# qiyunzhu/woltka

Measured on AMD Instinct MI355X. Metric: alignment records/sec classified, higher is better.
Workload: dtype u8; 1 GPU; synthetic SAM text of 50M reads x <=16 hits (10.50 GB) resident in HBM, 2M-node taxonomy, ranks phylum,genus,species: device tokenizer per 64 MB block + one weighted histogram per sample (the kernels of `woltka classify`, host link left out); records_per_gpu=250034804, reads_per_gpu=50000000

## Files before the change

### include/woltka_hip_measure.h

```cpp
#ifndef WOLTKA_HIP_MEASURE_H
#define WOLTKA_HIP_MEASURE_H
#include "woltka_hip.h"
#ifdef __cplusplus
extern "C" {
#endif

int wk_tune(wk_ctx* ctx, const char* name, int64_t value);

int wk_timer_begin(wk_ctx* ctx);
int wk_timer_end(wk_ctx* ctx);
int wk_timer_ms(wk_ctx* ctx, double* ms);
int wk_profile_kernels(wk_ctx* ctx, int enable);
int wk_last_kernel_ms(wk_ctx* ctx, const char* family, double* ms);

int wk_text_upload(wk_ctx* ctx, const char* text, int64_t begin, int64_t stop);
int wk_text_clear(wk_ctx* ctx);
int wk_dtok_fused_counts(wk_ctx* ctx, int64_t* done, int64_t* handed_back);
int wk_ordinal_chunk_counts(wk_ctx* ctx, int64_t* sorted, int64_t* gathered);
int wk_h2d_rate(wk_ctx* ctx, int64_t bytes, int reps, double* bytes_per_s);

#ifdef __cplusplus
}
#endif
#endif
```

### woltka_amd/_native.py

```python
import ctypes as C
import os
from fractions import Fraction

import numpy as np

_HERE = os.path.dirname(os.path.abspath(__file__))
LIB_PATH = os.environ.get('WOLTKA_HIP_LIB') or os.path.join(
    _HERE, 'libwoltka_hip.so')

ABI_VERSION = 5
OK, E_HIP, E_ARG, E_STATE, E_CAPACITY, E_RANGE, E_TABLE_FULL = (
    0, -1, -2, -3, -4, -5, -6)
KEY_FEATURE_BITS, KEY_GROUP_BITS, KEY_K_BITS, KEY_JOB_BITS = 28, 21, 12, 3
MAX_JOBS, MAX_K = 8, 4095
FEATURE_UNASSIGNED, MAX_FEATURE = 0x0FFFFFFF, 0x0FFFFFFE
MODE_NONE, MODE_FREE, MODE_RANK = 0, 1, 2
F_UNIQ, F_ABOVE, F_SUBOK, F_UNASSIGNED, F_SIZED = 1, 2, 4, 8, 16
ASSIGN_NONE, ASSIGN_MULTI, ASSIGN_EMPTY = -1, -2, -3
SUBJ_IS_SET, SUBJ_INDEXED, GROUP_UNIFORM = 1, 2, 4
MAX_RANK_SLOTS = MAX_JOBS * 4

SYMBOLS = (
    'wk_abi_version', 'wk_build_id', 'wk_device_count', 'wk_device_pci_bus_id',
    'wk_create', 'wk_destroy',
# ... 19 lines not shown
    'wk_tok_fetch', 'wk_tok_fetch_packed', 'wk_tok_set_subject_map',
    'wk_tok_read', 'wk_tok_trim', 'wk_tok_sam_span', 'wk_tok_span', 'wk_tok_set_header_state',
    'wk_dtok_format',
    'wk_dtok_copy', 'wk_dtok_copy_ahead', 'wk_dtok_copy_wait',
    'wk_dtok_copy_drop', 'wk_dtok_subject_map', 'wk_dtok_ahead_room', 'wk_dtok_text_back', 'wk_dtok_expect', 'wk_dtok_scan', 'wk_dtok_emit', 'wk_dtok_stage_hits', 'wk_dtok_stage_hits_append',
    'wk_dtok_scan_emit', 'wk_dtok_scan_emit_begin', 'wk_dtok_scan_emit_end',
    'wk_dtok_keep_reads', 'wk_readmap_tables',
    'wk_cover_begin', 'wk_dtok_cover_append', 'wk_cover_add',
    'wk_cover_finish', 'wk_cover_fetch', 'wk_cover_reset',
    'wk_dtok_readmap',
    'wk_dtok_readmap_fetch', 'wk_strata_load', 'wk_strata_labels',
    'wk_strata_groups', 'wk_strata_clear',
    'wk_demux_begin', 'wk_demux_pending', 'wk_demux_register',
    'wk_dtok_stage_reads', 'wk_demux_fetch', 'wk_dtok_stage_hits_demux',
    'wk_dtok_stage_reads_strata', 'wk_chunk_groups',
    'wk_dtok_stage_reads_plain', 'wk_classify_staged_keep',
    'wk_readmap_reads_tables', 'wk_dtok_readmap_reads',
    'wk_tok_subjects',
    'wk_tok_new_subjects', 'wk_tok_fetch_groups', 'wk_tok_strata_clear',
    'wk_tok_strata_load', 'wk_tok_strata_labels', 'wk_tok_strata_select',
    'wk_tok_strata_swap', 'wk_format_readmap',
    'wk_tok_fetch_samples', 'wk_tok_new_samples', 'wk_preorder',
    'wk_hier_create', 'wk_hier_destroy', 'wk_hier_last_error',
    'wk_hier_add_text', 'wk_hier_update', 'wk_hier_finish', 'wk_hier_arrays',
    'wk_hier_root', 'wk_hier_lookup', 'wk_hier_node_names', 'wk_hier_get',
    'wk_hier_size', 'wk_hier_keys', 'wk_hier_ranks',
    'wk_coords_parse', 'wk_coords_error', 'wk_coords_sizes',
    'wk_coords_fetch', 'wk_coords_free',
    'wk_gz_bound', 'wk_gz_member', 'wk_crc32', 'wk_gz_inflate_members',
    'wk_inflate_members_device', 'wk_dtok_inflate_ahead',
    'wk_gz_walk_members',
    'wk_gunzip_open', 'wk_gunzip_read', 'wk_gunzip_error', 'wk_gunzip_close',
    'wk_text_upload', 'wk_text_clear', 'wk_h2d_rate',
    'wk_dtok_fused_counts', 'wk_ordinal_chunk_counts')


class Job(C.Structure):
    _fields_ = [('mode', C.c_int32), ('rank_slot', C.c_int32),
                ('flags', C.c_uint32), ('_pad', C.c_uint32),
                ('major', C.c_double)]


class Stats(C.Structure):
    _fields_ = [('n_reads', C.c_int64), ('n_records', C.c_int64),
                ('n_pairs', C.c_int64), ('table_used', C.c_int64)]


_lib = None


def load_library():
    global _lib
    if _lib is not None:
        return _lib
    if not os.path.isfile(LIB_PATH):
        raise RuntimeError(
            f'{LIB_PATH} is missing: build it with `python -c "import '
            '__graft_entry__ as g; g.build()"` (hipcc --offload-arch=gfx950). '
            'There is no CPU fallback.')
    lib = C.CDLL(LIB_PATH)
    p = C.c_void_p
    i32p, i64p, u32p, u64p = (C.POINTER(C.c_int32), C.POINTER(C.c_int64),
                              C.POINTER(C.c_uint32), C.POINTER(C.c_uint64))
    proto = {
        'wk_abi_version': (C.c_int, []),
        'wk_build_id': (C.c_char_p, []),
        'wk_device_count': (C.c_int, []),
# ... 188 lines not shown
                                     i64p, C.POINTER(C.c_uint8), C.c_int64]),
        'wk_hier_finish': (C.c_int, [p, i64p, i32p]),
        'wk_hier_arrays': (C.c_int, [p, i32p, i32p, i32p, i32p]),
        'wk_hier_root': (C.c_int, [p, i32p]),
        'wk_hier_lookup': (C.c_int, [p, C.c_char_p, i64p, C.c_int64, i32p]),
        'wk_hier_node_names': (C.c_int, [p, i32p, C.c_int64, C.c_void_p,
                                         C.c_int64, i64p]),
        'wk_hier_get': (C.c_int, [p, C.c_int, C.c_char_p, C.c_int64,
                                  C.c_void_p, C.c_int64, i64p]),
        'wk_hier_size': (C.c_int64, [p, C.c_int]),
        'wk_hier_keys': (C.c_int, [p, C.c_int, C.c_void_p, C.c_int64, i64p]),
        'wk_hier_ranks': (C.c_int, [p, C.c_void_p, C.c_int64, i64p, i64p]),
        'wk_coords_parse': (C.c_int, [C.c_void_p, C.c_int64, C.POINTER(p)]),
        'wk_coords_error': (C.c_char_p, [p]),
        'wk_coords_sizes': (C.c_int, [p, i32p, i32p, i64p, i64p,
                                      C.POINTER(C.c_int)]),
        'wk_coords_fetch': (C.c_int, [p, i32p, i32p, i32p, i32p, C.c_void_p,
                                      i64p, C.c_void_p, i64p]),
        'wk_coords_free': (None, [p]),
        'wk_gz_bound': (C.c_int64, [C.c_int64]),
        'wk_gz_member': (C.c_int64, [C.c_void_p, C.c_int64, C.c_void_p,
                                     C.c_int64]),
        'wk_crc32': (C.c_uint32, [C.c_uint32, C.c_void_p, C.c_int64]),
        'wk_gz_inflate_members': (C.c_int64, [C.c_void_p, i64p, i64p, C.c_int64,
                                              C.c_void_p, i64p, C.c_int]),
        'wk_gunzip_open': (p, [C.c_char_p, C.c_int, C.c_char_p, C.c_size_t]),
        'wk_gunzip_read': (C.c_int64, [p, C.c_void_p, C.c_int64]),
        'wk_gunzip_error': (C.c_char_p, [p]),
        'wk_gunzip_close': (None, [p]),
        'wk_text_upload': (C.c_int, [p, C.c_void_p, C.c_int64, C.c_int64]),
        'wk_text_clear': (C.c_int, [p]),
        'wk_dtok_fused_counts': (C.c_int, [p, i64p, i64p]),
        'wk_ordinal_chunk_counts': (C.c_int, [p, i64p, i64p]),
        'wk_h2d_rate': (C.c_int, [p, C.c_int64, C.c_int,
                                  C.POINTER(C.c_double)]),
    }
    for name, (res, args) in proto.items():
        fn = getattr(lib, name)
        fn.restype = res
        fn.argtypes = args
    if lib.wk_abi_version() != ABI_VERSION:
        raise RuntimeError('libwoltka_hip.so ABI version mismatch')
    _lib = lib
    return lib


def _arr(a, dtype):
    return np.ascontiguousarray(a, dtype=dtype)


def _ptr(a, ctype):
    return None if a is None else a.ctypes.data_as(C.POINTER(ctype))


def device_pci_bus_id(device):
    buf = C.create_string_buffer(64)
    if load_library().wk_device_pci_bus_id(int(device), buf, 64) != OK:
        raise RuntimeError('no such HIP device')
    return buf.value.decode()


def decode_keys(keys):
    keys = np.asarray(keys, dtype=np.uint64)
    feat = (keys & np.uint64((1 << KEY_FEATURE_BITS) - 1)).astype(np.int64)
    grp = ((keys >> np.uint64(KEY_FEATURE_BITS)) &
           np.uint64((1 << KEY_GROUP_BITS) - 1)).astype(np.int64)
# ... 385 lines not shown
            return False
        started = C.c_int(0)
        self._check(self._lib.wk_dtok_scan_emit_begin(
            self._h, tok._h, C.c_void_p(raw.ctypes.data), int(begin),
            int(stop), C.byref(started)))
        return bool(started.value)

    def dtok_scan_emit_end(self):
        n, st = C.c_int64(0), C.c_int(1)
        a, b = C.c_int64(0), C.c_int64(0)
        self._check(self._lib.wk_dtok_scan_emit_end(
            self._h, C.byref(n), C.byref(st), C.byref(a), C.byref(b)))
        return (n.value, a.value) if st.value == 0 else None

    def text_upload(self, buf, begin, stop):
        raw = np.frombuffer(memoryview(buf), dtype=np.uint8)
        self._check(self._lib.wk_text_upload(
            self._h, C.c_void_p(raw.ctypes.data), int(begin), int(stop)))

    def text_clear(self):
        self._check(self._lib.wk_text_clear(self._h))

    def ordinal_chunk_counts(self):
        a, b = C.c_int64(0), C.c_int64(0)
        self._check(self._lib.wk_ordinal_chunk_counts(self._h, C.byref(a),
                                                      C.byref(b)))
        return a.value, b.value

    def dtok_fused_counts(self):
        a, b = C.c_int64(0), C.c_int64(0)
        self._check(self._lib.wk_dtok_fused_counts(self._h, C.byref(a),
                                                   C.byref(b)))
        return a.value, b.value

    def h2d_rate(self, nbytes=64 << 20, reps=32):
        out = C.c_double(0.0)
        self._check(self._lib.wk_h2d_rate(self._h, int(nbytes), int(reps),
                                          C.byref(out)))
        return out.value

    def dtok_format(self, fmt):
        self._check(self._lib.wk_dtok_format(self._h, Tokenizer.FORMATS[fmt]))

    def dtok_emit(self):
        a, b, st = C.c_int64(0), C.c_int64(0), C.c_int(1)
        self._check(self._lib.wk_dtok_emit(self._h, C.byref(a), C.byref(b),
                                           C.byref(st)))
        return st.value, a.value, b.value

    def cover_begin(self, cap_rows=0):
        self._check(self._lib.wk_cover_begin(self._h, int(cap_rows)))

    def cover_reset(self):
        self._check(self._lib.wk_cover_reset(self._h))

    def cover_fetch(self):
        n = C.c_int64(0)
        self._check(self._lib.wk_cover_finish(self._h, C.byref(n)))
        subj, beg, end = (np.empty(n.value, dtype=np.int32) for _ in range(3))
        self._check(self._lib.wk_cover_fetch(
            self._h, _ptr(subj, C.c_int32), _ptr(beg, C.c_int32),
            _ptr(end, C.c_int32), n.value))
        return subj, beg, end

    def _cover_spill(self, spill):
        if spill is None:
# ... 959 lines not shown
```

### woltka_amd/csrc/wk_dtok_fused.hpp

```cpp
#pragma once
#include "wk_dtok.hpp"
#include "wk_dtok_neighbour.hpp"
#include "wk_dtok_planes.hpp"
#include "wk_dtok_rounds.hpp"

namespace wk {

constexpr uint32_t kFzThreads = 512;
constexpr uint32_t kFzWaves = kFzThreads / kWave;
constexpr uint32_t kFzTile = 16384;
constexpr uint32_t kFzBack = 1024;
constexpr uint32_t kFzFwd = 3072;
constexpr uint32_t kFzWin = kFzTile + kFzBack + kFzFwd;
constexpr uint32_t kFzChunks = kFzWin / 16 + 1;
constexpr uint32_t kFzRounds = kFrMaxRounds;
static_assert(kFrChunks * 16u == kFzWin && kFrTailChunk + 1u == kFzChunks && kFrWaves == kFzWaves && kFrWave == kWave,
              "the dealing covers the window");
constexpr uint32_t kFzLines = 1024;
constexpr uint32_t kFzStreams = 4;
constexpr uint32_t kFzCap = 1024;
static_assert(kFzCap >= kFzLines, "a window's records fit an empty buffer");
static_assert(kFzWin + 32 < 65536, "window offsets fit 16 bits");
constexpr uint32_t kFzCarry = 256;
static_assert(kFzCarry + kFzLines <= kFpMaxLines && kFzThreads % kWave == 0, "a window's owned lines fit the planes, a wave's lines one word");

constexpr uint32_t kDtokSpill = 64;

struct FusedArgs {
    const unsigned char* text;
    uint32_t n;
    uint32_t open_end;
    uint32_t span;
    const struct DictSlot8* dict8;
    const uint4* names16;
    uint32_t dict_mask;
    const unsigned char* arena;
    uint2* unknown;
    uint32_t unknown_cap;
    DtokState* state;
    DtokState* host_state;
    const unsigned long long* backup_prev;
    unsigned long long* backup_next;
    uint32_t* host_seq;
    uint32_t seq;
    StreamSet streams;
    const int32_t* submap;
    uint32_t n_submap;
    uint32_t ablate;
};

static_assert(sizeof(DtokState) % 8 == 0, "the packed totals are aligned");
__device__ __forceinline__ unsigned long long* fz_totals(DtokState* state) { return reinterpret_cast<unsigned long long*>(state + 1); }

__global__ void dtok_fused_begin_kernel(unsigned long long* __restrict__ backup, const unsigned long long* __restrict__ cursor, DtokState* state) {
    if (threadIdx.x < (uint32_t)kMaxStreams) backup[threadIdx.x] = cursor[threadIdx.x];
    if (threadIdx.x == 0) {
        *state = DtokState{0u, 0u, 0ull, 0ull, 0ull, 0u, 0u};
        *fz_totals(state) = 0ull;
    }
}

template <int kCtrl, int kRowMask>
__device__ __forceinline__ uint32_t fz_dpp_add(uint32_t v) {
    return v + (uint32_t)__builtin_amdgcn_update_dpp(0, (int)v, kCtrl, kRowMask, 0xF, false);
}
__device__ __forceinline__ uint32_t fz_wave_scan(uint32_t v) {
    static_assert(kWave == 64, "four rows of sixteen lanes");
    v = fz_dpp_add<0x111, 0xF>(v);
    v = fz_dpp_add<0x112, 0xF>(v);
    v = fz_dpp_add<0x114, 0xF>(v);
    v = fz_dpp_add<0x118, 0xF>(v);
    v = fz_dpp_add<0x142, 0xA>(v);
    v = fz_dpp_add<0x143, 0xC>(v);
    return v;
}
__device__ __forceinline__ uint32_t fz_last_lane(uint32_t v) { return (uint32_t)__builtin_amdgcn_readlane((int)v, kWave - 1); }
__device__ __forceinline__ uint32_t fz_wave_sum(uint32_t v) { return fz_last_lane(fz_wave_scan(v)); }
__device__ __forceinline__ unsigned long long fz_first_lane64(unsigned long long v) {
    return ((unsigned long long)(uint32_t)__builtin_amdgcn_readfirstlane((int)(uint32_t)(v >> 32)) << 32) |
           (uint32_t)__builtin_amdgcn_readfirstlane((int)(uint32_t)v);
}
// ... 127 lines not shown
constexpr uint32_t kFiSubj = (1u << 23) - 1u;
constexpr uint32_t kFiMateShift = 24;
constexpr uint32_t kFiMapped = 1u << 26;
constexpr uint32_t kFiStart = 1u << 27;
constexpr uint32_t kFiUndecided = 1u << 28;
constexpr uint32_t kFiExcl = 1u << 29;
constexpr uint32_t kFiDropped = 1u << 30;
constexpr uint32_t kFiRead = kFiMapped | (3u << kFiMateShift);
constexpr uint32_t kFiKey = kFiRead | kFiSubj;
constexpr uint32_t kFzPad = 8;
static_assert(kFwWave == kWave && kFwWaves == kFzWaves, "the line pass's dealing is this workgroup's");

__device__ __forceinline__ uint32_t fz_octet(uint32_t z_lo, uint32_t z_hi) { return (((z_lo >> 7) | (z_hi >> 3)) * 0x00204081u >> 21) & 255u; }

__device__ __forceinline__ uint32_t fz_newlines16(uint4 v) {
    return fz_octet(fz_marks32(v.x, 0x0A0A0A0Au), fz_marks32(v.y, 0x0A0A0A0Au)) | (fz_octet(fz_marks32(v.z, 0x0A0A0A0Au), fz_marks32(v.w, 0x0A0A0A0Au)) << 8);
}

__device__ __forceinline__ uint32_t fz_tabs32(const unsigned char* p, unsigned long long* q0 = nullptr, unsigned long long* q1 = nullptr) {
    unsigned long long w[4];
#pragma unroll
    for (uint32_t i = 0; i < 4; ++i) w[i] = fz_load64(p + 8u * i);
    uint32_t m = 0;
#pragma unroll
    for (uint32_t i = 0; i < 4; ++i)
        m |= fz_octet(fz_marks32((uint32_t)w[i], 0x09090909u), fz_marks32((uint32_t)(w[i] >> 32), 0x09090909u)) << (8u * i);
    if (q0) {
        *q0 = w[0];
        *q1 = w[1];
    }
    return m;
}

template <bool kMeasure>
__device__ __forceinline__ void dtok_fused_body(const FusedArgs& a) {
    __shared__ __attribute__((aligned(16))) unsigned char txt[kFzChunks * 16 + 32];
    __shared__ uint16_t ls[kFzLines + 2];
    __shared__ uint16_t f_qn[kFzLines];
    __shared__ __attribute__((aligned(16))) uint32_t info_[kFzPad + kFzCarry + kFzLines + kFzPad + 8];
    __shared__ uint32_t carry[kFzCarry];
    __shared__ unsigned long long planes[kFpPlanes][kFpWords];
    __shared__ uint32_t rbuf[kFzStreams][kFzCap];
    __shared__ unsigned long long fill_packed;
    static_assert(kFzStreams <= 4 && kFzCap + kFzThreads < 65536, "four 16-bit counts");
    __shared__ unsigned long long gbase[kFzStreams];
    __shared__ uint32_t wtot[kFzWaves];
    __shared__ unsigned long long gbase_out[kMaxStreams];
    __shared__ unsigned long long wg_totals;
    __shared__ uint32_t own[5];
    __shared__ uint32_t wg_flags;
    uint32_t* const info = info_ + kFzPad + kFzCarry;

    const uint32_t tid = threadIdx.x, lane = tid & (kWave - 1), wave = tid / kWave;
    const uint32_t wave_s = (uint32_t)__builtin_amdgcn_readfirstlane((int)wave);
    const uint32_t n_streams = a.streams.n_streams;
    const uint32_t ablate = kMeasure ? a.ablate : 0u;
    const int32_t* const submap = a.submap;
    unsigned long long fill = 0ull;
    if (tid == 0) fill_packed = 0ull;
    if (tid < 4u) reinterpret_cast<uint32_t*>(txt + kFrTailChunk * 16u)[tid] = 0u;
    if (tid == 0) wg_flags = 0u;
    if (tid == 0) wg_totals = 0ull;
    uint32_t my_flags = 0, my_reads = 0, my_lines = 0;
    const uint32_t text_end = a.n + (a.open_end ? 1u : 0u);

    auto flush_all = [&](unsigned long long have, bool last) {
        __syncthreads();
        if (wave_s == 0u) {
            uint32_t xl = lane;
            asm volatile("" : "+v"(xl));
            if (xl < n_streams) {
                const uint32_t cnt = (ablate & 64u) ? 0u : (uint32_t)(have >> (16u * xl)) & 0xFFFFu;
                unsigned long long base = 0ull;
                if (cnt) {
                    base = atomicAdd(&a.streams.cursor[xl], (unsigned long long)cnt);
                    if (base + cnt > a.streams.cap) atomicOr(&wg_flags, kDtokSpill);
                }
                gbase[xl] = base;
            }
        }
        __syncthreads();
        for (uint32_t k = 0; k < n_streams; ++k) {
            const uint32_t cnt = (ablate & 64u) ? 0u : (uint32_t)(have >> (16u * k)) & 0xFFFFu;
            const unsigned long long base = gbase[k];
            for (uint32_t i = tid; i < cnt; i += kFzThreads)
                if (base + i < a.streams.cap) a.streams.out[k][base + i] = rbuf[k][i];
        }
        if (last) return;
        __syncthreads();
    };

    const uint32_t t0 = blockIdx.x * a.span;
    const uint32_t t1 = a.n - t0 > a.span ? t0 + a.span : a.n;
    const uint32_t span_w1 = fr_min_end(t1, kFzFwd, text_end);
    uint32_t wpos = t0 >= kFzBack ? t0 - kFzBack : 0u;
    uint32_t mode = 0u;
    uint32_t counted = t0;
    bool wide = false;
    uint32_t nc = 0u;
    uint32_t cq_pos = 0u, cq_len = 0u;
    const uint32_t max_trips = a.span / 16u + 2u;
    for (uint32_t trip = 0;; ++trip) {
        if (trip >= max_trips) {
            my_flags |= kDtokSpill;
            break;
        }
        const uint32_t w0 = wpos & ~15u;
        const uint32_t lead = wpos - w0;
        const uint32_t w1 = fr_min_end(mode == 0u ? t0 : w0, mode == 0u ? kFzTile + kFzFwd : kFzWin, wide ? text_end : span_w1);
        const bool to_end = w1 == text_end;
        const bool last_win = wide || w1 == span_w1;
        __syncthreads();
        uint32_t ws = wave_s;
        asm volatile("" : "+s"(ws));
        if (ws == 0u) {
            uint32_t xl = lane;
            asm volatile("" : "+v"(xl));
            if (xl < 5u) own[xl] = xl < 2u ? 0xFFFFFFFFu : 0u;
            if (xl < kFzPad) info[-(int32_t)nc - 1 - (int32_t)xl] = kFiStart;
        }
        for (uint32_t i = tid; i < nc; i += kFzThreads) info[(int32_t)i - (int32_t)nc] = carry[i];

        const uint32_t wave_c0 = fr_first_chunk(wave_s), ws_c0 = fr_first_chunk(ws), wave_rounds = fr_rounds(ws);
        uint4 v[kFzRounds];
#pragma unroll
        for (uint32_t r = 0; r < kFzRounds; ++r) {
            const uint32_t p = w0 + (wave_c0 + r * kWave + lane) * 16u;
            v[r] = make_uint4(0u, 0u, 0u, 0u);
            if (r < wave_rounds && p < a.n && p < w1) v[r] = fz_load_stream(a.text + p);
        }
        uint32_t marks[kFzRounds];
        uint32_t nl_packed = 0;
        bool blank = false;
        const uint32_t in_lo = max(wpos, counted), in_hi = min(min(w1, a.n), t1);
#pragma unroll
        for (uint32_t r = 0; r < kFzRounds; ++r) {
            const uint32_t c = wave_c0 + r * kWave + lane;
            const uint32_t p = w0 + c * 16u;
            marks[r] = 0u;
            if (r >= wave_rounds) continue;
            const uint32_t rp0 = w0 + (ws_c0 + r * kWave) * 16u;
            const bool interior = rp0 >= in_lo && fr_fits(rp0, kWave * 16u, in_hi);
            *reinterpret_cast<uint4*>(txt + c * 16u) = v[r];
            if (interior) {
                const uint32_t m = fr_chunk_marks(fz_newlines16(v[r]), &blank);
                const uint32_t cnt = (uint32_t)__popc(m);
                my_lines += cnt;
                marks[r] = m;
                nl_packed |= fr_pack(cnt, r);
            } else if (p < w1) {
                uint32_t m = fz_newlines16(v[r]);
                if (p + 16u > a.n) m &= p >= a.n ? 0u : (1u << (a.n - p)) - 1u;
                if (p >= counted && p < t1) my_lines += (uint32_t)__popc(m);
                if (a.n - p < 16u) m |= a.open_end << (a.n - p);
                if (p + 16u > w1) m &= (1u << (w1 - p)) - 1u;
                if (p < wpos) m &= ~((1u << (wpos - p)) - 1u);
                m = fr_chunk_marks(m, &blank);
                marks[r] = m;
                nl_packed |= fr_pack((uint32_t)__popc(m), r);
            }
        }
        if (blank && !(ablate & 16u)) my_flags |= kDtokShortLine;
        const uint32_t nl_inc = fz_wave_scan(nl_packed);
        const uint32_t nl_wave = fz_last_lane(nl_inc);
        if (lane == 0) wtot[wave] = fr_total(nl_wave);
        __syncthreads();
        uint32_t before = 0, total_nl = 0;
#pragma unroll
        for (uint32_t w = 0; w < kFzWaves; ++w) {
            const uint32_t t = (uint32_t)__builtin_amdgcn_readfirstlane((int)wtot[w]);
            before += w < ws ? t : 0u;
            total_nl += t;
        }
        const bool too_many = total_nl + 1u > kFzLines || (ablate & (32u | 512u));
        if (too_many) {
            if (!(ablate & 512u)) my_flags |= kDtokSpill;
        } else {
            if (tid == 0) ls[0] = (uint16_t)lead;
            uint32_t line = before;
#pragma unroll
            for (uint32_t r = 0; r < kFzRounds; ++r) {
                if (r >= wave_rounds) continue;
                const uint32_t c = wave_c0 + r * kWave + lane;
                uint32_t at = line + fr_unpack(nl_inc, r) - (uint32_t)__popc(marks[r]);
                uint32_t m = marks[r];
                while (m) {
                    const uint32_t b = (uint32_t)__ffs((int)m) - 1u;
                    ls[++at] = (uint16_t)(c * 16u + b + 1u);
                    m &= m - 1u;
                }
                line += fr_unpack(nl_wave, r);
            }
        }
        __syncthreads();
        const uint32_t trail = too_many ? wpos : w0 + (uint32_t)__builtin_amdgcn_readfirstlane((int)(uint32_t)ls[total_nl]);
        if (!too_many && last_win && trail >= t0 && trail < t1) my_flags |= kDtokSpill;
        const uint32_t first_line = mode != 0u || w0 == 0u ? 0u : 1u;
        const uint32_t n_lines = too_many ? 0u : total_nl;
        if (tid == 0 && first_line) info[0] = 0u;

        const bool first_starts = nc == 0u && (mode == 1u || wpos == 0u);
        for (uint32_t k0 = first_line; k0 < n_lines; k0 += kFwTrip) {
            const uint32_t k = fw_line(k0, wave, lane);
            const bool has = fw_has(k, first_line, n_lines), owner = !fw_witness(lane);
            uint32_t word = 0, s = 0, qn = 0, rb = 0, rn = 0;
            unsigned long long q0 = 0ull, q1 = 0ull;
            if (has) {
                s = ls[k];
                const uint32_t e = (uint32_t)ls[k + 1] - 1u;
                uint32_t tab[3] = {0, 0, 0}, nt = 0;
                if (!(ablate & 256u)) {
                    uint32_t m = fz_tabs32(txt + s, &q0, &q1);
                    if (e - s < 32u) m &= (1u << (e - s)) - 1u;
                    nt = min((uint32_t)__popc(m), 3u);
                    tab[0] = s + (uint32_t)__ffs((int)m) - 1u;
                    m &= m - 1u;
                    tab[1] = s + (uint32_t)__ffs((int)m) - 1u;
                    m &= m - 1u;
                    tab[2] = s + (uint32_t)__ffs((int)m) - 1u;
                    for (uint32_t p = s + 32u; nt < 3u && p < e; p += 32u) {
                        m = fz_tabs32(txt + p);
                        if (e - p < 32u) m &= (1u << (e - p)) - 1u;
                        for (; m && nt < 3u; m &= m - 1u) {
                            const uint32_t q = p + (uint32_t)__ffs((int)m) - 1u;
                            if (nt == 0u)
                                tab[0] = q;
                            else if (nt == 1u)
// ... 40 lines not shown
            prev.meta = (uint32_t)__builtin_amdgcn_update_dpp(0, (int)me.meta, 0x138 , 0xF, 0xF, false);
#pragma unroll
            for (uint32_t i = 0; i < 4; ++i) prev.b[i] = (uint32_t)__builtin_amdgcn_update_dpp(0, (int)me.b[i], 0x138, 0xF, 0xF, false);
            const uint32_t verdict = ((ablate & 8u) || (first_starts && k == first_line)) ? (uint32_t)kFnStarts : (uint32_t)fn_verdict(prev, me);
            const bool start = look && verdict == kFnStarts;
            const unsigned long long b_und = __ballot(look && verdict == kFnUndecided);
            if (lane == 0 && b_und != 0ull) own[4] = 1u;
            if (look) {
                int32_t sid = (ablate & 1u) ? (int32_t)(fz_load32(name + 4) % 1000u) : fz_probe_end(a, probe, name, rn, w0 + rb);
                bool excluded = false;
                if (submap && sid >= 0) {
                    if ((uint32_t)sid < a.n_submap) {
                        sid = submap[sid];
                        if (sid == kLineExcluded) {
                            excluded = true;
                            sid = 0;
                        }
                    } else {
                        my_flags |= kDtokSpill;
                        sid = -1;
                    }
                }
                word |= (start ? kFiStart : 0u) | (verdict == kFnUndecided ? kFiUndecided : 0u) | (excluded ? kFiExcl : 0u) |
                        (sid < 0 ? kFiSubj : ((uint32_t)sid & kFiSubj));
            }
            if (has && owner) info[k] = word;
            const unsigned long long b_all = __ballot(start), b_in = __ballot(start && w0 + s < t1), b_out = b_all & ~b_in;
            if (lane == 0 && b_all) {
                if (b_in) atomicMin(&own[0], k + (uint32_t)__builtin_ctzll(b_in));
                if (b_out) atomicMin(&own[1], k + (uint32_t)__builtin_ctzll(b_out));
                atomicMax(&own[2], k + 63u - (uint32_t)__builtin_clzll(b_all));
            }
        }
        __syncthreads();
        if (__builtin_amdgcn_readfirstlane((int)own[4])) {
        for (uint32_t k0 = first_line; k0 < n_lines; k0 += kFzThreads) {
            const uint32_t k = k0 + tid;
            const uint32_t mk = k < n_lines ? info[k] : 0u;
            const bool und = (mk & kFiUndecided) != 0u;
            bool start = false;
            if (__ballot(und) != 0ull) {
                if (und) {
                    uint32_t j = k;
                    bool found = false;
                    while (j > first_line) {
                        --j;
                        if (info[j] & kFiMapped) {
                            found = true;
                            break;
                        }
                    }
                    if (found)
                        start = f_qn[j] != f_qn[k] || !fz_same(txt + ls[k], txt + ls[j], f_qn[k]);
                    else if (nc)
                        start = f_qn[k] != cq_len || !fz_same(txt + ls[k], a.text + cq_pos, cq_len);
                    else if (mode == 1u || wpos == 0u)
                        start = true;
                    else
                        start = fz_starts_run_slow(a.text, w0 + ls[first_line], txt + ls[k], f_qn[k]);
                }
            }
            if (mk & kFiUndecided) {
                info[k] = (mk & ~kFiUndecided) | (start ? kFiStart : 0u);
                if (start) {
                    atomicMin(&own[w0 + ls[k] < t1 ? 0 : 1], k);
                    atomicMax(&own[2], k);
                }
// ... 40 lines not shown
            next = trail;
            next_mode = 2u;
            more = trail > wpos && trail < t1;
            if (trail <= wpos) my_flags |= kDtokSpill;
        }
        if (put_aside) {
            if (tid == 0) {
                uint32_t c = nc;
                for (uint32_t k = first_line; k < n_lines; ++k) {
                    const uint32_t w = info[k];
                    if (w & kFiMapped) {
                        if (c < kFzCarry) carry[c] = w & ~kFiDropped;
                        ++c;
                    }
                }
                own[3] = c;
            }
            __syncthreads();
            nc_next = (uint32_t)__builtin_amdgcn_readfirstlane((int)own[3]);
            if (nc_next > kFzCarry || trail <= wpos) {
                my_flags |= kDtokSpill;
                nc_next = 0u;
            } else {
                if (nc == 0u) {
                    cq_pos = wpos;
                    cq_len = (uint32_t)__builtin_amdgcn_readfirstlane((int)(uint32_t)f_qn[0]);
                }
                next = trail;
                next_mode = 2u;
                more = true;
                again = last_win;
            }
        }
        for (int32_t k0 = ka; k0 < kb; k0 += (int32_t)kFzThreads) {
            const int32_t k = k0 + (int32_t)tid;
            const uint32_t mk = k < kb ? info[k] : 0u;
            const bool mapped = (mk & kFiMapped) != 0u, excl = mapped && (mk & kFiExcl);
            if (excl) {
                int32_t j = k;
                while (!(info[j] & kFiStart)) --j;
                atomicOr(&info[j], kFiDropped);
            }
            bool dup = false;
            if (mapped && !excl && !(mk & kFiStart) && !(ablate & 2u)) {
                bool done = false;
                for (int32_t j = k; !done; j -= 8) {
                    uint32_t w[8];
#pragma unroll
                    for (uint32_t i = 0; i < 8; ++i) w[i] = info[j - 1 - (int32_t)i];
#pragma unroll
                    for (uint32_t i = 0; i < 8; ++i) {
                        dup |= !done && ((w[i] ^ mk) & kFiKey) == 0u;
                        done |= (w[i] & kFiStart) != 0u;
                    }
                }
            }
            const bool first = mapped && !excl && !dup;
            const uint32_t mate = (mk >> kFiMateShift) & 3u;
            const uint32_t wi = (uint32_t)__builtin_amdgcn_readfirstlane((int)((uint32_t)(k0 - ka) / kWave + wave));
            const bool put = lane == 0 && wi < kFpWords;
            const unsigned long long p_start = __ballot(mapped && (mk & kFiStart));
            if (put) planes[kFpStart][wi] = p_start;
#pragma unroll
            for (uint32_t m = 0; m < 4; ++m) {
                const unsigned long long p_first = __ballot(first && mate == m);
                if (put) planes[kFpFirst + m][wi] = p_first;
            }
        }
        __syncthreads();
        for (int32_t k0 = ka; k0 < kb; k0 += (int32_t)kFzThreads) {
            const int32_t k = k0 + (int32_t)tid;
            bool rec = false;
            uint32_t word = 0, sl = 0, at = 0;
            const uint32_t li = (uint32_t)(k - ka);
            const uint32_t mk = k < kb ? info[k] : 0u;
            const unsigned long long* const mine = planes[kFpFirst + ((mk >> kFiMateShift) & 3u)];
            if (k < kb && ((mine[li / 64u] >> (li % 64u)) & 1ull) && !(ablate & 4u)) {
                uint32_t pos = 0, size = 1;
                bool dropped = (mk & kFiStart) && (mk & kFiDropped);
                if (!(ablate & (2u | 128u))) {
                    const FpRead r = fp_read(planes[kFpStart], mine, li, (uint32_t)(kb - ka));
                    pos = r.pos;
                    size = r.size;
                    dropped = (info[ka + (int32_t)r.head] & kFiDropped) != 0u;
                }
                if (size > (uint32_t)WK_WEIGHT_MAX_K) my_flags |= kDtokBigRead;
                const uint32_t s = mk & kFiSubj;
                if (s != kFiSubj && !dropped) {
                    rec = true;
                    word = s | ((pos & 15u) << kWordSubjBits) | ((size & 31u) << kWordSizeShift);
                    sl = s / kSliceBins;
                    if (sl >= n_streams) sl = n_streams - 1u;
                    my_reads += pos == 0u ? 1u : 0u;
                }
            }
            {
                unsigned long long add = 0;
                uint32_t mine_before = 0;
                for (uint32_t s2 = 0; s2 < n_streams; ++s2) {
                    const unsigned long long m = __ballot(rec && sl == s2);
                    add |= (unsigned long long)__popcll(m) << (16u * s2);
                    if (rec && sl == s2) mine_before = (uint32_t)__popcll(m & ((1ull << lane) - 1ull));
                }
                if (add) {
                    unsigned long long base = 0;
                    if (lane == 0) base = atomicAdd(&fill_packed, add);
                    base = fz_first_lane64(base);
                    at = (uint32_t)(base >> (16u * sl)) & 0xFFFFu;
                    at += mine_before;
                }
            }
            __syncthreads();
            unsigned long long now = fz_first_lane64(fill_packed);
            static_assert(kFzCap + 0x7BFFu == 0x7FFFu && 2u * kFzCap + kFzThreads + 0x7BFFu < 0x10000u, "the full test");
            if ((now + 0x7BFF7BFF7BFF7BFFull) & 0x8000800080008000ull) {
                flush_all(fill, false);
                at -= (uint32_t)(fill >> (16u * sl)) & 0xFFFFu;
                now -= fill;
                if (tid == 0) fill_packed = now;
            }
            if (rec) rbuf[sl][at] = word;
            fill = now;
            if (k0 + (int32_t)kFzThreads < kb) __syncthreads();
        }
        if (!more) break;
        wpos = next;
        mode = next_mode;
        wide = again;
        nc = nc_next;
        counted = w1;
    }
    if (my_flags) atomicOr(&wg_flags, my_flags);
    {
        const uint32_t reads_w = fz_wave_sum(my_reads), lines_w = fz_wave_sum(my_lines);
        const unsigned long long t = ((unsigned long long)lines_w << 32) | reads_w;
        if (lane == 0 && t) atomicAdd(&wg_totals, t);
    }
    flush_all(fill, true);
    __syncthreads();
    if (tid == 0) {
        if (wg_totals) __hip_atomic_fetch_add(fz_totals(a.state), wg_totals, __ATOMIC_RELAXED, __HIP_MEMORY_SCOPE_AGENT);
        if (wg_flags) atomicOr(&a.state->flags, wg_flags);
        __threadfence();
        own[0] = atomicAdd(&a.state->done, 1u) == gridDim.x - 1u ? 1u : 0u;
    }
    __syncthreads();
    if (own[0]) {
        __threadfence();
        uint32_t xt = tid;
        asm volatile("" : "+v"(xt));
        if (xt < (uint32_t)kMaxStreams) {
            const unsigned long long cur = __hip_atomic_load(&a.streams.cursor[xt], __ATOMIC_RELAXED, __HIP_MEMORY_SCOPE_AGENT);
            a.backup_next[xt] = cur;
            gbase_out[xt] = xt < n_streams ? cur - a.backup_prev[xt] : 0ull;
        }
        __syncthreads();
        if (tid == 0) {
            DtokState st{};
            st.flags = __hip_atomic_load(&a.state->flags, __ATOMIC_RELAXED, __HIP_MEMORY_SCOPE_AGENT);
            st.n_unknown = __hip_atomic_load(&a.state->n_unknown, __ATOMIC_RELAXED, __HIP_MEMORY_SCOPE_AGENT);
            const unsigned long long totals = __hip_atomic_load(fz_totals(a.state), __ATOMIC_RELAXED, __HIP_MEMORY_SCOPE_AGENT);
            for (uint32_t k = 0; k < (uint32_t)kMaxStreams; ++k) st.n_out += gbase_out[k];
            st.n_reads = totals & 0xFFFFFFFFull;
            st.n_lines = totals >> 32;
            *a.host_state = st;
            *a.state = DtokState{0u, 0u, 0ull, 0ull, 0ull, 0u, 0u};
            *fz_totals(a.state) = 0ull;
            __threadfence_system();
            if (a.host_seq) __hip_atomic_store(a.host_seq, a.seq, __ATOMIC_RELEASE, __HIP_MEMORY_SCOPE_SYSTEM);
        }
    }
}

__global__ void __launch_bounds__(kFzThreads) __attribute__((amdgpu_waves_per_eu(6, 6))) dtok_fused_kernel(FusedArgs a) {
    dtok_fused_body<false>(a);
}
__global__ void __launch_bounds__(kFzThreads) __attribute__((amdgpu_waves_per_eu(6, 6))) dtok_fused_measure_kernel(FusedArgs a) {
    dtok_fused_body<true>(a);
}

}
```

### woltka_amd/csrc/woltka_hip.hip

```cpp
#include <hip/hip_runtime.h>

#include <algorithm>
#include <atomic>
#include <ctime>
#include <chrono>
#include <cstdarg>
#include <cstdio>
#include <cstdlib>
#include <cstring>
#include <map>
#include <new>
#include <mutex>
#include <string>
#include <vector>

#include "../../include/woltka_hip.h"
#include "../../include/woltka_hip_measure.h"
#include "wk_classify.hpp"
#include "wk_cover.hpp"
#include "wk_device.hpp"
#include "wk_dtok.hpp"
#include "wk_demux.hpp"
#include "wk_strata_reads.hpp"
#include "wk_dtok_fused.hpp"
// ... 252 lines not shown
    std::vector<wk_job> w_jobs;
    int32_t w_group = 0;
    bool w_open = false;
    struct HostReg {
        const char* p;
        size_t n;
    };
    std::mutex reg_mu;
    std::vector<HostReg> regs;
    int w_mode = 0;
    bool w_mixed_entry = false;
    int rank_serial = 0;
    int free_per_cu = 2, free_threads = 1024, free_slots = 4096;
    int32_t max_gene_feature = 0;
    int use_range_log = 1;
    int words_keep = 0;
    static constexpr int kStageSlots = 8;
    hipEvent_t slot_ev[kStageSlots] = {};
    bool slot_busy[kStageSlots] = {};
    std::vector<void*> host_blocks;
    std::mutex host_mu;
    static constexpr int kTextBufs = 192;
    static constexpr int kSlabBufs = 16;
    static constexpr size_t kTextStride = ((size_t)66 << 20) + 256;
    DevBuf d_textslab[kTextBufs / kSlabBufs];
    enum : unsigned char { kBufFree = 0, kBufCopied = 1, kBufScanning = 2, kBufPending = 3 };
    TextBuf text_buf[kTextBufs];
    std::mutex copy_mu;
    std::mutex slab_mu;
    unsigned long long copy_seq_next = 1;
    unsigned long long* copy_newlines = nullptr;
    uint32_t* di_any_host = nullptr;
    DevBuf d_tiles, d_tile_off, d_lines, d_lsubj, d_lmeta, d_start, d_first, d_unknown, d_state, d_dict, d_dict2, d_names16, d_arena, d_submap;
    bool dt_mapped = false;
    bool dt_submap_on = false;
    bool dt_has_excl = false;
    uint32_t dt_submap_n = 0;
    DevBuf d_lbeg, d_lend, d_llen, d_lscan, d_gmap;
    bool dt_extra = false;
    DevBuf cv_key[2], cv_end[2], cv_reach, cv_hist, cv_tiles, cv_tile_off, cv_state, cv_stage[3];
    bool cv_open = false;
    int cv_cur = 0;
    int64_t cv_cap = 0;
    int64_t cv_cap_opt = 0;
    int64_t cv_tail = 0;
    int64_t cv_merged = 0;
    int64_t cv_ub = 0;
    bool cv_stale = false;
    CoverState cv_seen{};
    uint32_t cv_line_next = 0;
    struct ResidentText {
        const char* host;
        uint32_t n;
        unsigned char* dev;
        unsigned long long* tile_off;
        unsigned long long n_newlines;
    };
    std::vector<ResidentText> resident;
    DevBuf di_blob, di_meta, di_out, di_status;
    const unsigned char* dt_text = nullptr;
    int dt_fmt = 0;
    uint32_t dt_n = 0, dt_lines = 0, dt_dict_mask = 0;
    int32_t dt_dict_names = -1;
    const wk_tok* dt_dict_tok = nullptr;
    bool dt_ready = false;
    hipStream_t copy_stream = nullptr, count_stream = nullptr;
// ... 661 lines not shown
    if (const char* sm = getenv("WOLTKA_STRIPES_MIN"))
        if (sm[0]) c->stripes_min_hits = std::max<long long>(0, atoll(sm));
    *out = c;
    return WK_OK;
}

void wk_destroy(wk_ctx* c) {
    if (!c) return;
    DeviceGuard guard(c->device);
    if (c->stream) (void)hipStreamSynchronize(c->stream);
    DevBuf* bufs[] = {&c->nodes, &c->rank_code, &c->gene4, &c->g_grid, &c->g_first, &c->g_goff, &c->g_shift,
                      &c->tkeys, &c->tvals, &c->c_subj, &c->c_qoff, &c->c_group, &c->o_genome, &c->o_beg,
                      &c->o_end, &c->o_len, &c->o_hoff, &c->o_cnt, &c->o_ub, &c->o_first2, &c->o_poff, &c->o_pairs, &c->o_qoff,
                      &c->o_tile_sum, &c->o_tile_off, &c->scalars, &c->stat_block, &c->log, &c->subj_feat, &c->subj_rows, &c->dense_slab, &c->plog, &c->plog_cnt, &c->left_mask, &c->left_list, &c->first_slab, &c->w_slab, &c->w_hi, &c->w_invalid, &c->sz_rows, &c->sz_counts, &c->sz_scal, &c->lr_table, &c->c_rk[0], &c->c_rk[1], &c->rk_left[0], &c->rk_left[1], &c->rk_totals, &c->f_rank, &c->f_sparse, &c->f_dense, &c->w_renum, &c->f_log, &c->f_log_cnt, &c->f_partial, &c->f_part_used, &c->w_tmp, &c->assign_out, &c->fetch_k, &c->fetch_v};
    for (DevBuf* b : bufs) b->release();
    for (wk_ctx::StreamTables& T : c->st)
        for (DevBuf* b : {&T.dsparse, &T.dparent, &T.dself, &T.rnode, &T.subj_node, &T.subj_rank}) b->release();
    c->c_words.release();
    for (DevBuf* b : {&c->di_blob, &c->di_meta, &c->di_out, &c->di_status}) b->release();
    for (DevBuf& b : c->w_stream) b.release();
    c->w_wide.release();
    c->w_wide_plan.release();
    c->w_backup2.release();
    c->w_backup3.release();
    for (hipEvent_t& e : c->lag_ev)
        if (e) (void)hipEventDestroy(e);
    for (TextBuf& b : c->text_buf) {
        for (DevBuf* d : {&b.tiles, &b.tile_off, &b.di_comp, &b.di_meta, &b.di_status, &b.own}) d->release();
        for (hipEvent_t ev : {b.ev, b.ev0, b.evm})
            if (ev) (void)hipEventDestroy(ev);
    }
    for (DevBuf& slab : c->d_textslab) slab.release();
    for (DevBuf* b : {&c->d_tiles, &c->d_tile_off, &c->d_lines, &c->d_lsubj, &c->d_lmeta, &c->d_start, &c->d_first, &c->d_unknown, &c->d_lbeg, &c->d_lend, &c->d_llen, &c->d_lscan, &c->d_gmap,
                      &c->d_state, &c->d_dict, &c->d_dict2, &c->d_names16, &c->d_arena, &c->d_submap, &c->cv_key[0], &c->cv_key[1], &c->cv_end[0], &c->cv_end[1],
                      &c->cv_reach, &c->cv_hist, &c->cv_tiles, &c->cv_tile_off, &c->cv_state, &c->cv_stage[0], &c->cv_stage[1], &c->cv_stage[2],
                      &c->dx_tab, &c->dx_name_off, &c->dx_arena, &c->dx_group, &c->dx_met, &c->dx_pend, &c->dx_pend_list, &c->dx_state, &c->dx_lsamp, &c->dx_out, &c->dx_rsamp,
                      &c->rr_off, &c->rr_text, &c->rr_flags})
        b->release();
    for (wk_ctx::ResidentText& r : c->resident) {
        (void)hipFree(r.dev);
        (void)hipFree(r.tile_off);
    }
    c->resident.clear();
    for (void* hp : c->host_blocks) (void)hipHostFree(hp);
    if (c->host_back) (void)hipHostFree(c->host_back);
    for (const wk_ctx::HostReg& r : c->regs) (void)hipHostUnregister(const_cast<char*>(r.p));
    c->regs.clear();
    if (c->di_any_host) (void)hipHostFree(c->di_any_host);
    if (c->copy_stream) (void)hipStreamDestroy(c->copy_stream);
    if (c->count_stream) (void)hipStreamDestroy(c->count_stream);
    if (c->res_ev) (void)hipEventDestroy(c->res_ev);
    for (hipEvent_t ev : c->slot_ev)
        if (ev) (void)hipEventDestroy(ev);
    for (DevBuf& b : c->rank_tab) b.release();
    for (auto& kv : c->ktimers)
        if (kv.second.b) (void)hipEventDestroy(kv.second.b);
    if (c->kt_step) (void)hipEventDestroy(c->kt_step);
    if (c->t0) (void)hipEventDestroy(c->t0);
    if (c->t1) (void)hipEventDestroy(c->t1);
    if (c->stream) (void)hipStreamDestroy(c->stream);
    delete c;
}

int wk_device_name(const wk_ctx* c, char* buf, size_t cap) {
    if (!c || !buf || cap == 0) return WK_E_ARG;
    snprintf(buf, cap, "%s (%s, %d CUs)", c->prop.name, c->prop.gcnArchName, c->prop.multiProcessorCount);
    return WK_OK;
// ... 2233 lines not shown
    if (e == hipSuccess) e = hipStreamCreateWithFlags(&st, hipStreamNonBlocking);
    if (e == hipSuccess) e = hipEventCreate(&e0);
    if (e == hipSuccess) e = hipEventCreate(&e1);
    for (int i = 0; i < 2 && e == hipSuccess; ++i) e = hipMemcpyAsync(d[i], h[i], (size_t)bytes, hipMemcpyHostToDevice, st);
    if (e == hipSuccess) e = hipEventRecord(e0, st);
    for (int i = 0; i < reps && e == hipSuccess; ++i) e = hipMemcpyAsync(d[i & 1], h[i & 1], (size_t)bytes, hipMemcpyHostToDevice, st);
    if (e == hipSuccess) e = hipEventRecord(e1, st);
    if (e == hipSuccess) e = hipEventSynchronize(e1);
    float ms = 0.f;
    if (e == hipSuccess) e = hipEventElapsedTime(&ms, e0, e1);
    cleanup();
    if (e != hipSuccess) {
        (void)hipGetLastError();
        return fail(c, WK_E_HIP, "wk_h2d_rate: %s", hipGetErrorString(e));
    }
    *bytes_per_s = ms > 0.f ? (double)bytes * reps / (ms * 1e-3) : 0.0;
    return WK_OK;
}

int wk_ordinal_chunk_counts(wk_ctx* c, int64_t* sorted, int64_t* gathered) {
    if (!c || !sorted || !gathered) return WK_E_ARG;
    *sorted = c->chunks_sorted;
    *gathered = c->chunks_gathered;
    return WK_OK;
}

int wk_dtok_fused_counts(wk_ctx* c, int64_t* done, int64_t* handed_back) {
    if (!c || !done || !handed_back) return WK_E_ARG;
    *done = c->fused_blocks;
    *handed_back = c->fused_fallbacks;
    return WK_OK;
}

int wk_text_clear(wk_ctx* c) {
    if (!c) return WK_E_ARG;
    DeviceGuard guard(c->device);
    for (wk_ctx::ResidentText& r : c->resident) {
        (void)hipFree(r.dev);
        (void)hipFree(r.tile_off);
    }
    c->resident.clear();
    return WK_OK;
}

int wk_dtok_subject_map(wk_ctx* c, const int32_t* map, int32_t n) {
    if (!c || n < 0 || (n > 0 && !map)) return WK_E_ARG;
    DeviceGuard guard(c->device);
    c->dt_submap_on = map != nullptr;
    if (map && n == 0) HIP_TRY(c, c->d_submap.reserve(64));
    bool excl = false;
    if (n > 0) {
        for (int32_t i = 0; i < n; ++i) {
            if (map[i] == kLineExcluded)
                excl = true;
            else if (map[i] < 0)
                return fail(c, WK_E_ARG, "a subject map holds subject indices (or -4: excluded)");
        }
        HIP_TRY(c, hipStreamSynchronize(c->stream));
        const int rc = upload(c, c->d_submap, map, (size_t)n * 4);
        if (rc) return rc;
        HIP_TRY(c, hipStreamSynchronize(c->stream));
    }
    c->dt_submap_n = (uint32_t)n;
    c->dt_has_excl = excl;
    return WK_OK;
}
// ... 40 lines not shown
static bool fused_eligible(const wk_ctx* c, const wk_tok* tok) {
    return c->use_fused && c->dt_fmt == WK_FMT_SAM && c->w_open && c->w_mode == 0 && !c->dt_keep_reads &&
           wkx_tok_n_names(tok) < (1 << 23) - 1;
}

static int fused_launch(wk_ctx* c, const StreamSet& streams, const unsigned char* text, uint32_t n, bool open_end, int ring, int host_slot,
                        uint32_t seq) {
    static_assert(sizeof(DtokState) <= 128 && wk_ctx::kBackBytes >= 132, "the slot's second half holds the block's sequence number");
    FusedArgs fa{};
    const unsigned grid = fused_spans(c, n, &fa.span);
    if (fa.span % 16u) return fail(c, WK_E_ARG, "spans of the one-kernel tokenizer are multiples of 16 bytes");
    HIP_TRY(c, dtok_scratch_reserve(c));
    for (int i = 0; i < 3; ++i) HIP_TRY(c, fz_bk(c, i).reserve(kMaxStreams * 8));
    fa.text = text;
    fa.n = n;
    fa.open_end = open_end ? 1u : 0u;
    fa.dict8 = c->d_dict2.as<DictSlot8>();
    fa.names16 = c->d_names16.as<uint4>();
    fa.dict_mask = c->dt_dict_mask;
    fa.arena = c->d_arena.as<unsigned char>();
    fa.unknown = c->d_unknown.as<uint2>();
    fa.unknown_cap = (uint32_t)(c->d_unknown.cap / 8);
    fa.state = c->d_state.as<DtokState>();
    unsigned char* slot = c->host_back + (size_t)host_slot * wk_ctx::kBackBytes;
    fa.host_state = reinterpret_cast<DtokState*>(slot);
    fa.backup_prev = fz_bk(c, ring).as<unsigned long long>();
    fa.backup_next = fz_bk(c, (ring + 1) % 3).as<unsigned long long>();
    fa.host_seq = seq ? reinterpret_cast<uint32_t*>(slot + 128) : nullptr;
    fa.seq = seq;
    fa.streams = streams;
    fa.submap = c->dt_submap_on ? c->d_submap.as<int32_t>() : nullptr;
    fa.n_submap = c->dt_submap_n;
    fa.ablate = c->fused_ablate;
    c->w_counts_known = false;
    KernelTimer* kf = ktimer_begin(c, "dtok_fused");
    if (!c->fz_chain)
        hipLaunchKernelGGL(dtok_fused_begin_kernel, dim3(1), dim3(64), 0, c->stream, fz_bk(c, ring).as<unsigned long long>(),
                           (const unsigned long long*)streams.cursor, fa.state);
    if (c->fused_ablate != 0u)
        hipLaunchKernelGGL(dtok_fused_measure_kernel, dim3(grid), dim3(kFzThreads), 0, c->stream, fa);
    else
        hipLaunchKernelGGL(dtok_fused_kernel, dim3(grid), dim3(kFzThreads), 0, c->stream, fa);
    ktimer_end(c, kf);
    HIP_TRY(c, hipGetLastError());
    return WK_OK;
}

static uint32_t fz_kept(wk_ctx* c, const DtokState& st, uint32_t n, bool open_end) {
    const uint32_t lines = (uint32_t)st.n_lines + (open_end ? 1u : 0u);
    c->dt_lines = lines;
    c->dt_lpb = (double)lines / (double)n;
    c->fused_streak = true;
    c->fz_back_streak = 0;
    ++c->fused_blocks;
    return lines;
}

static void fz_handed_back(wk_ctx* c) {
    c->fused_streak = false;
    c->fz_chain = false;
    ++c->fused_fallbacks;
    c->fz_back_streak = std::min(c->fz_back_streak + 1, 6);
    if (c->fz_back_streak >= 2) c->fz_skip = 1 << (c->fz_back_streak - 1);
}

struct ScanBlock {
// ... 2312 lines not shown
```

Baseline: 16.95 billion records/s.

## Prefetch next window's text during plane writes in fused tokenizer and add timeline probe

The fused tokenizer kernel now issues the global loads for the next window before the plane-writing phase of the current window. This lets text fetch latency overlap with compute instead of being paid at the top of each trip. It also adds an optional wall-clock timeline instrumentation path, active only in the measure kernel under an ablate flag, plus a host API to read it back. Keeping the prefetched registers live across the loop may raise register pressure. The added s_waitcnt before the prefetch may also serialize outstanding memory operations.

```diff
diff --git a/include/woltka_hip_measure.h b/include/woltka_hip_measure.h
--- a/include/woltka_hip_measure.h
+++ b/include/woltka_hip_measure.h
@@ -16,6 +16,9 @@
 int wk_text_upload(wk_ctx* ctx, const char* text, int64_t begin, int64_t stop);
 int wk_text_clear(wk_ctx* ctx);
 int wk_dtok_fused_counts(wk_ctx* ctx, int64_t* done, int64_t* handed_back);
+int wk_dtok_fused_timeline(wk_ctx* ctx, uint64_t* out, int64_t cap,
+                           int64_t* n_wgs, int64_t* words_per_wg,
+                           int64_t* every);
 int wk_ordinal_chunk_counts(wk_ctx* ctx, int64_t* sorted, int64_t* gathered);
 int wk_h2d_rate(wk_ctx* ctx, int64_t bytes, int reps, double* bytes_per_s);
 
diff --git a/woltka_amd/_native.py b/woltka_amd/_native.py
--- a/woltka_amd/_native.py
+++ b/woltka_amd/_native.py
@@ -75,7 +75,8 @@
     'wk_gz_walk_members',
     'wk_gunzip_open', 'wk_gunzip_read', 'wk_gunzip_error', 'wk_gunzip_close',
     'wk_text_upload', 'wk_text_clear', 'wk_h2d_rate',
-    'wk_dtok_fused_counts', 'wk_ordinal_chunk_counts')
+    'wk_dtok_fused_counts', 'wk_ordinal_chunk_counts',
+    'wk_dtok_fused_timeline')
 
 
 class Job(C.Structure):
@@ -330,6 +331,8 @@
         'wk_text_clear': (C.c_int, [p]),
         'wk_dtok_fused_counts': (C.c_int, [p, i64p, i64p]),
         'wk_ordinal_chunk_counts': (C.c_int, [p, i64p, i64p]),
+        'wk_dtok_fused_timeline': (C.c_int, [p, C.c_void_p, C.c_int64, i64p,
+                                             i64p, i64p]),
         'wk_h2d_rate': (C.c_int, [p, C.c_int64, C.c_int,
                                   C.POINTER(C.c_double)]),
     }
@@ -781,6 +784,17 @@
         self._check(self._lib.wk_dtok_fused_counts(self._h, C.byref(a),
                                                    C.byref(b)))
         return a.value, b.value
+
+    def dtok_fused_timeline(self):
+        n, w, ev = C.c_int64(0), C.c_int64(0), C.c_int64(0)
+        self._check(self._lib.wk_dtok_fused_timeline(
+            self._h, None, 0, C.byref(n), C.byref(w), C.byref(ev)))
+        out = np.zeros((n.value, w.value), dtype=np.uint64)
+        if out.size:
+            self._check(self._lib.wk_dtok_fused_timeline(
+                self._h, out.ctypes.data, out.size, C.byref(n), C.byref(w),
+                C.byref(ev)))
+        return out, ev.value
 
     def h2d_rate(self, nbytes=64 << 20, reps=32):
         out = C.c_double(0.0)
diff --git a/woltka_amd/csrc/wk_dtok_fused.hpp b/woltka_amd/csrc/wk_dtok_fused.hpp
--- a/woltka_amd/csrc/wk_dtok_fused.hpp
+++ b/woltka_amd/csrc/wk_dtok_fused.hpp
@@ -23,6 +23,24 @@
 static_assert(kFzWin + 32 < 65536, "window offsets fit 16 bits");
 constexpr uint32_t kFzCarry = 256;
 static_assert(kFzCarry + kFzLines <= kFpMaxLines && kFzThreads % kWave == 0, "a window's owned lines fit the planes, a wave's lines one word");
+
+constexpr uint32_t kFzAblateTop = 2048, kFzAblateTimeline = 4096;
+constexpr uint32_t kFzTlEvery = 64, kFzTlWindows = 24, kFzTlHead = 4, kFzTlPer = 12;
+constexpr uint32_t kFzTlWords = kFzTlHead + kFzTlWindows * kFzTlPer;
+enum : uint32_t {
+    kFzTlBarrier = 0,
+    kFzTlTop,
+    kFzTlText,
+    kFzTlStaged,
+    kFzTlNumbered,
+    kFzTlProbed,
+    kFzTlLines,
+    kFzTlAhead,
+    kFzTlPlanes,
+    kFzTlEnd,
+    kFzTlInfo,
+};
+static_assert(kFzTlInfo < kFzTlPer, "a window's words");
 
 constexpr uint32_t kDtokSpill = 64;
 
@@ -47,6 +65,7 @@
     const int32_t* submap;
     uint32_t n_submap;
     uint32_t ablate;
+    unsigned long long* timeline;
 };
 
 static_assert(sizeof(DtokState) % 8 == 0, "the packed totals are aligned");
@@ -240,7 +259,7 @@
     return m;
 }
 
-template <bool kMeasure>
+template <bool kMeasure, bool kAhead>
 __device__ __forceinline__ void dtok_fused_body(const FusedArgs& a) {
     __shared__ __attribute__((aligned(16))) unsigned char txt[kFzChunks * 16 + 32];
     __shared__ uint16_t ls[kFzLines + 2];
@@ -263,6 +282,18 @@
     const uint32_t wave_s = (uint32_t)__builtin_amdgcn_readfirstlane((int)wave);
     const uint32_t n_streams = a.streams.n_streams;
     const uint32_t ablate = kMeasure ? a.ablate : 0u;
+    const bool ahead = kMeasure ? !(ablate & kFzAblateTop) : kAhead;
+    unsigned long long* tl = nullptr;
+    if (kMeasure && (ablate & kFzAblateTimeline) && a.timeline != nullptr && blockIdx.x % kFzTlEvery == 0u)
+        tl = a.timeline + (size_t)(blockIdx.x / kFzTlEvery) * kFzTlWords;
+    auto stamp = [&](uint32_t word) {
+        if (kMeasure && tl != nullptr && tid == 0) tl[word] = wall_clock64();
+    };
+    auto stamp_window = [&](uint32_t trip_, uint32_t which) {
+        if (kMeasure && trip_ < kFzTlWindows) stamp(kFzTlHead + trip_ * kFzTlPer + which);
+    };
+    stamp(0);
+    if (kMeasure && tl != nullptr && tid == 0) tl[3] = blockIdx.x;
     const int32_t* const submap = a.submap;
     unsigned long long fill = 0ull;
     if (tid == 0) fill_packed = 0ull;
@@ -308,6 +339,19 @@
     uint32_t nc = 0u;
     uint32_t cq_pos = 0u, cq_len = 0u;
     const uint32_t max_trips = a.span / 16u + 2u;
+    auto window_end = [&](uint32_t w0_, uint32_t mode_, bool wide_) {
+        return fr_min_end(mode_ == 0u ? t0 : w0_, mode_ == 0u ? kFzTile + kFzFwd : kFzWin, wide_ ? text_end : span_w1);
+    };
+    auto load_window = [&](uint4 (&v_)[kFzRounds], uint32_t w0_, uint32_t w1_, uint32_t c0_, uint32_t rounds_) {
+#pragma unroll
+        for (uint32_t r = 0; r < kFzRounds; ++r) {
+            const uint32_t p = w0_ + (c0_ + r * kWave + lane) * 16u;
+            v_[r] = make_uint4(0u, 0u, 0u, 0u);
+            if (r < rounds_ && p < a.n && p < w1_) v_[r] = fz_load_stream(a.text + p);
+        }
+    };
+    uint4 v[kFzRounds];
+    bool loaded = false;
     for (uint32_t trip = 0;; ++trip) {
         if (trip >= max_trips) {
             my_flags |= kDtokSpill;
@@ -315,10 +359,11 @@
         }
         const uint32_t w0 = wpos & ~15u;
         const uint32_t lead = wpos - w0;
-        const uint32_t w1 = fr_min_end(mode == 0u ? t0 : w0, mode == 0u ? kFzTile + kFzFwd : kFzWin, wide ? text_end : span_w1);
+        const uint32_t w1 = window_end(w0, mode, wide);
         const bool to_end = w1 == text_end;
         const bool last_win = wide || w1 == span_w1;
         __syncthreads();
+        stamp_window(trip, kFzTlBarrier);
         uint32_t ws = wave_s;
         asm volatile("" : "+s"(ws));
         if (ws == 0u) {
@@ -330,12 +375,12 @@
         for (uint32_t i = tid; i < nc; i += kFzThreads) info[(int32_t)i - (int32_t)nc] = carry[i];
 
         const uint32_t wave_c0 = fr_first_chunk(wave_s), ws_c0 = fr_first_chunk(ws), wave_rounds = fr_rounds(ws);
-        uint4 v[kFzRounds];
-#pragma unroll
-        for (uint32_t r = 0; r < kFzRounds; ++r) {
-            const uint32_t p = w0 + (wave_c0 + r * kWave + lane) * 16u;
-            v[r] = make_uint4(0u, 0u, 0u, 0u);
-            if (r < wave_rounds && p < a.n && p < w1) v[r] = fz_load_stream(a.text + p);
+        const bool loaded_here = loaded;
+        if (!loaded) load_window(v, w0, w1, wave_c0, wave_rounds);
+        if (kMeasure && tl != nullptr) {
+            stamp_window(trip, kFzTlTop);
+            __builtin_amdgcn_s_waitcnt(0x0F70);
+            stamp_window(trip, kFzTlText);
         }
         uint32_t marks[kFzRounds];
         uint32_t nl_packed = 0;
@@ -373,6 +418,7 @@
         const uint32_t nl_wave = fz_last_lane(nl_inc);
         if (lane == 0) wtot[wave] = fr_total(nl_wave);
         __syncthreads();
+        stamp_window(trip, kFzTlStaged);
         uint32_t before = 0, total_nl = 0;
 #pragma unroll
         for (uint32_t w = 0; w < kFzWaves; ++w) {
@@ -401,6 +447,7 @@
             }
         }
         __syncthreads();
+        stamp_window(trip, kFzTlNumbered);
         const uint32_t trail = too_many ? wpos : w0 + (uint32_t)__builtin_amdgcn_readfirstlane((int)(uint32_t)ls[total_nl]);
         if (!too_many && last_win && trail >= t0 && trail < t1) my_flags |= kDtokSpill;
         const uint32_t first_line = mode != 0u || w0 == 0u ? 0u : 1u;
@@ -507,7 +554,9 @@
                 atomicMax(&own[2], k + 63u - (uint32_t)__builtin_clzll(b_all));
             }
         }
-        __syncthreads();
+        stamp_window(trip, kFzTlProbed);
+        __syncthreads();
+        stamp_window(trip, kFzTlLines);
         if (__builtin_amdgcn_readfirstlane((int)own[4])) {
         for (uint32_t k0 = first_line; k0 < n_lines; k0 += kFzThreads) {
             const uint32_t k = k0 + tid;
@@ -614,6 +663,13 @@
                 again = last_win;
             }
         }
+        __builtin_amdgcn_s_waitcnt(0x0F70);
+        loaded = ahead && more;
+        if (loaded) {
+            const uint32_t w0n = next & ~15u;
+            load_window(v, w0n, window_end(w0n, next_mode, again), wave_c0, wave_rounds);
+        }
+        stamp_window(trip, kFzTlAhead);
         for (int32_t k0 = ka; k0 < kb; k0 += (int32_t)kFzThreads) {
             const int32_t k = k0 + (int32_t)tid;
             const uint32_t mk = k < kb ? info[k] : 0u;
@@ -650,6 +706,7 @@
             }
         }
         __syncthreads();
+        stamp_window(trip, kFzTlPlanes);
         for (int32_t k0 = ka; k0 < kb; k0 += (int32_t)kFzThreads) {
             const int32_t k = k0 + (int32_t)tid;
             bool rec = false;
@@ -705,6 +762,11 @@
             fill = now;
             if (k0 + (int32_t)kFzThreads < kb) __syncthreads();
         }
+        stamp_window(trip, kFzTlEnd);
+        if (kMeasure && tl != nullptr && tid == 0) {
+            tl[2] = trip + 1u;
+            if (trip < kFzTlWindows) tl[kFzTlHead + trip * kFzTlPer + kFzTlInfo] = mode | (loaded_here ? 16u : 0u) | (more ? 32u : 0u);
+        }
         if (!more) break;
         wpos = next;
         mode = next_mode;
@@ -752,13 +814,14 @@
             if (a.host_seq) __hip_atomic_store(a.host_seq, a.seq, __ATOMIC_RELEASE, __HIP_MEMORY_SCOPE_SYSTEM);
         }
     }
+    stamp(1);
 }
 
 __global__ void __launch_bounds__(kFzThreads) __attribute__((amdgpu_waves_per_eu(6, 6))) dtok_fused_kernel(FusedArgs a) {
-    dtok_fused_body<false>(a);
+    dtok_fused_body<false, true>(a);
 }
 __global__ void __launch_bounds__(kFzThreads) __attribute__((amdgpu_waves_per_eu(6, 6))) dtok_fused_measure_kernel(FusedArgs a) {
-    dtok_fused_body<true>(a);
-}
-
-}
+    dtok_fused_body<true, true>(a);
+}
+
+}
diff --git a/woltka_amd/csrc/woltka_hip.hip b/woltka_amd/csrc/woltka_hip.hip
--- a/woltka_amd/csrc/woltka_hip.hip
+++ b/woltka_amd/csrc/woltka_hip.hip
@@ -308,6 +308,8 @@
     unsigned long long* copy_newlines = nullptr;
     uint32_t* di_any_host = nullptr;
     DevBuf d_tiles, d_tile_off, d_lines, d_lsubj, d_lmeta, d_start, d_first, d_unknown, d_state, d_dict, d_dict2, d_names16, d_arena, d_submap;
+    DevBuf d_timeline;
+    uint32_t tl_wgs = 0;
     bool dt_mapped = false;
     bool dt_submap_on = false;
     bool dt_has_excl = false;
@@ -1035,7 +1037,7 @@
     }
     for (DevBuf& slab : c->d_textslab) slab.release();
     for (DevBuf* b : {&c->d_tiles, &c->d_tile_off, &c->d_lines, &c->d_lsubj, &c->d_lmeta, &c->d_start, &c->d_first, &c->d_unknown, &c->d_lbeg, &c->d_lend, &c->d_llen, &c->d_lscan, &c->d_gmap,
-                      &c->d_state, &c->d_dict, &c->d_dict2, &c->d_names16, &c->d_arena, &c->d_submap, &c->cv_key[0], &c->cv_key[1], &c->cv_end[0], &c->cv_end[1],
+                      &c->d_state, &c->d_timeline, &c->d_dict, &c->d_dict2, &c->d_names16, &c->d_arena, &c->d_submap, &c->cv_key[0], &c->cv_key[1], &c->cv_end[0], &c->cv_end[1],
                       &c->cv_reach, &c->cv_hist, &c->cv_tiles, &c->cv_tile_off, &c->cv_state, &c->cv_stage[0], &c->cv_stage[1], &c->cv_stage[2],
                       &c->dx_tab, &c->dx_name_off, &c->dx_arena, &c->dx_group, &c->dx_met, &c->dx_pend, &c->dx_pend_list, &c->dx_state, &c->dx_lsamp, &c->dx_out, &c->dx_rsamp,
                       &c->rr_off, &c->rr_text, &c->rr_flags})
@@ -3335,6 +3337,22 @@
     return WK_OK;
 }
 
+int wk_dtok_fused_timeline(wk_ctx* c, uint64_t* out, int64_t cap, int64_t* n_wgs, int64_t* words_per_wg, int64_t* every) {
+    if (!c || !n_wgs || !words_per_wg || !every || cap < 0 || (cap > 0 && !out)) return WK_E_ARG;
+    DeviceGuard guard(c->device);
+    if (!c->d_timeline.p) {
+        HIP_TRY(c, c->d_timeline.reserve((size_t)16 * kFzTlWords * 8));
+        HIP_TRY(c, hipMemsetAsync(c->d_timeline.p, 0, c->d_timeline.cap, c->stream));
+    }
+    *n_wgs = c->tl_wgs;
+    *words_per_wg = kFzTlWords;
+    *every = kFzTlEvery;
+    const int64_t have = (int64_t)c->tl_wgs * (int64_t)kFzTlWords, take = std::min(have, cap);
+    if (take > 0) HIP_TRY(c, hipMemcpyAsync(out, c->d_timeline.p, (size_t)take * 8, hipMemcpyDeviceToHost, c->stream));
+    HIP_TRY(c, hipStreamSynchronize(c->stream));
+    return WK_OK;
+}
+
 int wk_text_clear(wk_ctx* c) {
     if (!c) return WK_E_ARG;
     DeviceGuard guard(c->device);
@@ -3441,6 +3459,14 @@
     fa.submap = c->dt_submap_on ? c->d_submap.as<int32_t>() : nullptr;
     fa.n_submap = c->dt_submap_n;
     fa.ablate = c->fused_ablate;
+    fa.timeline = nullptr;
+    if (c->fused_ablate & kFzAblateTimeline) {
+        const uint32_t wgs = (grid + kFzTlEvery - 1u) / kFzTlEvery;
+        HIP_TRY(c, c->d_timeline.reserve((size_t)std::max(wgs, 16u) * kFzTlWords * 8));
+        HIP_TRY(c, hipMemsetAsync(c->d_timeline.p, 0, (size_t)wgs * kFzTlWords * 8, c->stream));
+        fa.timeline = c->d_timeline.as<unsigned long long>();
+        c->tl_wgs = wgs;
+    }
     c->w_counts_known = false;
     KernelTimer* kf = ktimer_begin(c, "dtok_fused");
     if (!c->fz_chain)
```

Result: faster. 17.50 billion records/s, median of 6 (+3.2%).
